# jedward225/MARL-HideAndSeek

Measured on AMD Instinct MI355X. Metric: world-steps/sec (agent-steps/sec derived) at 16K worlds, 1/2/4/8 GPU, higher is better.
Workload: dtype f32; 1 GPU; 16000 worlds/GPU x 2646 steps, 2 hiders + 2 seekers, sim_flags=0, rand_seed=0, random move actions in [-5,4] each step (scripts/benchmark.py args); worlds_per_gpu=16000, total_worlds=16000, agents_per_world=4

## Files before the change

### marl-hideandseek_amd/csrc/hs_k_observe.h

```cpp
#pragma once
#include "hs_state.h"
#include "hs_rays.h"

namespace hs {

constexpr int kObsWaves = 7;

constexpr int kRaysPerAgent = 46;
constexpr int obs_vis_base(int a) { return (a * 30 + 63) / 64 * 64; }
constexpr int obs_threads(int a) { return (obs_vis_base(a) + a * 16 + 63) / 64 * 64; }
constexpr int obs_max_agents(int nt) { int a = 1; while (a < kMaxAgents && obs_threads(a + 1) <= nt) ++a; return a; }
struct RayId { int agent, k; };
HSD RayId ray_id(int r, int visBase) {
    if (r < visBase) { const int i = r / 30; return {i, r - i * 30}; }
    const int rr = r - visBase;
    return {rr >> 4, 30 + (rr & 15)};
}

struct ObsStaged {
    WorldGeom g;
    float lin[kNumDSlots][3];
    float ang[kNumDSlots][3];
    int grab[kMaxAgents];
};

template <int NT>
struct ObsShared : ObsStaged {
    static constexpr int kMaxRays = NT, kAgents = obs_max_agents(NT);
    float rayD[kMaxRays][3];
    unsigned long long rayKey[kMaxRays];
    static constexpr int kWaves = NT / 64, kWavePairs = 64 * (kMaxBoxes + kMaxAgents - 1), kWaveRampPairs = 64 * kMaxRamps;
    unsigned short pairs[kWaves][kWavePairs];
    unsigned short rampPairs[kWaves][kWaveRampPairs];
    int nPairs[kWaves], nRampPairs[kWaves];
    unsigned present;
    alignas(16) float rel[kAgents][kNumDSlots][8];
    float fwd[kAgents][3], right[kAgents][3];
};

HSD void store_posvel(float *o, V3 p, V3 e, V3 l, V3 a) {
    o[0] = p.x; o[1] = p.y; o[2] = p.z; o[3] = e.x; o[4] = e.y; o[5] = e.z;
    o[6] = l.x; o[7] = l.y; o[8] = l.z; o[9] = a.x; o[10] = a.y; o[11] = a.z;
}

struct StageSeg { int rows, inner, stride, dst; };
enum { kStMeta, kStPos, kStRot, kStLin, kStAng, kStWall, kStPlane, kStGrab, kStSegs };
#define HS_ST_WORD(field) (int)(offsetof(ObsStaged, field) / 4)
#define HS_ST_GWORD(field) (int)((offsetof(ObsStaged, g) + offsetof(WorldGeom, field)) / 4)
constexpr StageSeg kStageSegs[kStSegs] = {
    {kNumDSlots, kNumDSlots, 1, HS_ST_GWORD(meta)},
    {3 * kNumDSlots, kNumDSlots, 3, HS_ST_GWORD(pos)},
    {4 * kNumDSlots, kNumDSlots, 4, HS_ST_GWORD(rot)},
    {3 * kNumDSlots, kNumDSlots, 3, HS_ST_WORD(lin)},
    {3 * kNumDSlots, kNumDSlots, 3, HS_ST_WORD(ang)},
    {4 * kMaxWalls, kMaxWalls, 4, HS_ST_GWORD(wall)},
    {4 * kMaxPlanes, kMaxPlanes, 4, HS_ST_GWORD(plane)},
    {kMaxAgents, kMaxAgents, 1, HS_ST_WORD(grab)},
};
constexpr int stage_seg_start(int k) { int f = 0; for (int j = 0; j < k; ++j) f += kStageSegs[j].rows; return f; }
constexpr int stage_seg_of(int f) { int k = 0; while (k + 1 < kStSegs && stage_seg_start(k + 1) <= f) ++k; return k; }
constexpr int kStageWords = stage_seg_start(kStSegs);
constexpr int kStagedWords = (int)(sizeof(ObsStaged) / 4);
struct StageTable { unsigned short dst[kStageWords]; };
constexpr StageTable make_stage_table() {
    StageTable t = {};
    int f = 0;
    for (int k = 0; k < kStSegs; ++k)
        for (int r = 0; r < kStageSegs[k].rows; ++r)
            t.dst[f++] = (unsigned short)((kStageSegs[k].dst + (r % kStageSegs[k].inner) * kStageSegs[k].stride + r / kStageSegs[k].inner) * 4);
    return t;
}
constexpr bool stage_table_covers() {
    const StageTable t = make_stage_table();
    int hits[kStagedWords] = {};
    for (int f = 0; f < kStageWords; ++f) {
        if (t.dst[f] % 4 != 0 || t.dst[f] / 4 >= kStagedWords) return false;
        ++hits[t.dst[f] / 4];
    }
    for (int w = 0; w < kStagedWords; ++w)
        if (hits[w] != (w == HS_ST_GWORD(numWalls) || w == HS_ST_GWORD(numPlanes) ? 0 : 1)) return false;
    return true;
}
static_assert(stage_table_covers(), "the staging table must write every staged word of ObsStaged exactly once");
static_assert(kStageWords == kNumDSlots + 3 * (3 * kNumDSlots) + 4 * kNumDSlots + 4 * kMaxWalls + 4 * kMaxPlanes + kMaxAgents,
              "the staging table moves the words of the per-column loops it replaced");
static_assert(kStagedWords == kStageWords + 2 && sizeof(ObsStaged) % 4 == 0, "ObsStaged holds the staged words and the two counts");
static_assert(kStageSegs[kStMeta].rows == decltype(SimState::bmeta)::kRows && kStageSegs[kStPos].rows == decltype(SimState::bpos)::kRows &&
              kStageSegs[kStRot].rows == decltype(SimState::brot)::kRows && kStageSegs[kStLin].rows == decltype(SimState::blin)::kRows &&
              kStageSegs[kStAng].rows == decltype(SimState::bang)::kRows && kStageSegs[kStWall].rows == decltype(SimState::walls)::kRows &&
              kStageSegs[kStPlane].rows == decltype(SimState::planes)::kRows && kStageSegs[kStGrab].rows == decltype(SimState::grabOther)::kRows,
              "every staged source row lies inside its column");
#undef HS_ST_WORD
#undef HS_ST_GWORD
__device__ const StageTable kStageTable = make_stage_table();

template <int NT>
HSD unsigned stage_world(const SimState &S, int ps, ObsShared<NT> &sh, int tid) {
    typedef unsigned __attribute__((may_alias)) word_t;
    const char *const arena = reinterpret_cast<const char *>(S.bpos.p);
    const void *const cols[kStSegs] = {S.bmeta.p, S.bpos.p, S.brot.p, S.blin.p, S.bang.p, S.walls.p, S.planes.p, S.grabOther.p};
    unsigned K[kStSegs];
#pragma unroll
    for (int k = 0; k < kStSegs; ++k)
        K[k] = (unsigned)(reinterpret_cast<const char *>(cols[k]) - arena) +
               (((unsigned)(ps >> 3) * kStageSegs[k].rows - stage_seg_start(k)) * kTile + (ps & 7)) * 4u;
    constexpr int kTrips = (kStageWords + NT - 1) / NT;
    unsigned v[kTrips], d[kTrips];
#pragma unroll
    for (int t = 0; t < kTrips; ++t) {
        const int f = tid + t * NT;
        const int lo = t * NT, hi = (t + 1) * NT < kStageWords ? (t + 1) * NT - 1 : kStageWords - 1;
        unsigned k = K[stage_seg_of(lo)];
#pragma unroll
        for (int s = 1; s < kStSegs; ++s)
            if (stage_seg_start(s) > lo && stage_seg_start(s) <= hi) k = f >= stage_seg_start(s) ? K[s] : k;
        v[t] = 0; d[t] = 0;
        if ((t + 1) * NT <= kStageWords || f < kStageWords) {
            v[t] = *reinterpret_cast<const word_t *>(arena + (size_t)(k + (unsigned)f * (kTile * 4u)));
            d[t] = kStageTable.dst[f];
        }
    }
    static_assert(kStageSegs[kStMeta].rows <= 64 && stage_seg_start(kStMeta) == 0, "the metas are staged by wave 0 in its first trip");
    const unsigned present = (unsigned)__ballot(tid < kNumDSlots && v[0] != 0);
    char *const dst = reinterpret_cast<char *>(static_cast<ObsStaged *>(&sh));
#pragma unroll
    for (int t = 0; t < kTrips; ++t)
        if ((t + 1) * NT <= kStageWords || tid + t * NT < kStageWords) *reinterpret_cast<word_t *>(dst + d[t]) = v[t];
    if (tid < NT / 64) { sh.nPairs[tid] = 0; sh.nRampPairs[tid] = 0; }
    return present;
}

HSD unsigned long long ray_key(float t, int id) { return ((unsigned long long)__float_as_uint(t) << 32) | (unsigned)id; }
constexpr unsigned kKeyMiss = 0xffffffffu;

template <int NT>
__global__ void __launch_bounds__(NT) __attribute__((amdgpu_waves_per_eu(kObsWaves, kObsWaves))) k_observe(SimState S) {
    __shared__ ObsShared<NT> sh;
    const int tid = threadIdx.x;
#ifdef HS_PHASE_TIMING
    long long otk = wall_clock64();
    long long *const oacc = S.phaseTicks + phase_ticks_obs_base(S.N) + (blockIdx.x & 1023) * 16;
#define HS_OTICK(i) { const long long now_ = wall_clock64(); if ((tid & 63) == 0) atomicAdd((unsigned long long *)&oacc[i], (unsigned long long)(now_ - otk)); otk = now_; }
#else
#define HS_OTICK(i)
#endif
    const int blk = blockIdx.x;
    int oct = ((blk >> 6) << 3) + (blk & 7);
    const int noct = (S.N + kTile - 1) / kTile;
    if (oct >= noct) return;
    if (step_serve(S) != kGroupAll) {
        if (oct >= *group_count(S, step_ring(S), step_serve(S))) return;
        oct = oct_list(S, step_ring(S), step_serve(S), noct)[oct];
    }
    const int p = oct * kTile + ((blk >> 3) & 7);
    const int4 hdr = S.slotHdr[p];
    const int A = S.A;
    const int visBase = obs_vis_base(A);
    const RayId myRay = ray_id(tid, visBase);
    float lidarS = 0.f, lidarC = 0.f;
    if (tid < visBase) { lidarS = S.lidarSinCos[myRay.k]; lidarC = S.lidarSinCos[30 + myRay.k]; }
    const unsigned present = stage_world<NT>(S, p, sh, tid);
    const int w = hdr.x;
    if (w < 0) return;
    if (tid == 0) { sh.g.numWalls = hdr.y & 255; sh.g.numPlanes = (hdr.y >> 8) & 255; sh.present = present; }
    const int counts = hdr.z;
    const int teams = hdr.w;
    const int step = hdr.y >> 16;
    __syncthreads();
    const WorldGeom &g = sh.g;
    const int nAgents = cnt_agents(counts), nBoxes = cnt_boxes(counts), nRamps = cnt_ramps(counts);
    HS_OTICK(0)
    static_assert(kNumDSlots - 1 == 16 && ObsShared<NT>::kAgents * 16 <= NT - 8, "item = agent * 16 + other body; the last 8 lanes have no item");
    for (int item = tid; item < nAgents * 16; item += NT) {
        const int i = item >> 4, ob = item & 15;
        const int b = ob + (ob >= kAgentSlot0 + i ? 1 : 0);
        const int m = g.meta[b];
        if (m == 0) continue;
        const V3 mo = g.g_pos(kAgentSlot0 + i) - g.g_pos(b);
        const V3 ol = qrot(qinv(g.g_rot(b)), mo);
        float *e = sh.rel[i][b];
        e[0] = mo.x; e[1] = mo.y; e[2] = mo.z;
        e[3] = dot(mo, mo) - obj_bound_r2(meta_obj(m));
        e[4] = ol.x; e[5] = ol.y; e[6] = ol.z;
    }
    for (int i = tid - (NT - 8); i >= 0 && i < nAgents; i += NT) {
        const Q rot = g.g_rot(kAgentSlot0 + i);
        const V3 f = qrot(rot, {0.f, 1.f, 0.f}), rt = qrot(rot, {1.f, 0.f, 0.f});
        sh.fwd[i][0] = f.x; sh.fwd[i][1] = f.y; sh.fwd[i][2] = f.z;
        sh.right[i][0] = rt.x; sh.right[i][1] = rt.y; sh.right[i][2] = rt.z;
    }
    __syncthreads();
    HS_OTICK(1)

    for (int r = tid; r < NT; r += NT) {
        const int i = myRay.agent, k = myRay.k;
        sh.rayKey[r] = ray_key(-1.f, kKeyMiss);
        if (i >= nAgents) continue;
        const int slot = kAgentSlot0 + i;
        const V3 o = g.g_pos(slot);
        const V3 fwd = {sh.fwd[i][0], sh.fwd[i][1], sh.fwd[i][2]};
        V3 d; float tmax;
        if (k < 30) {
            const V3 right = {sh.right[i][0], sh.right[i][1], sh.right[i][2]};
            const float s = lidarS, c = lidarC;
            d = normalize(right * c + fwd * s);
            tmax = 200.f;
        } else {
            const int e = k - 30;
            int tslot; bool present;
            if (e < kMaxBoxes) { tslot = kBoxSlot0 + e; present = e < nBoxes; }
            else if (e < kMaxBoxes + kMaxRamps) { tslot = kRampSlot0 + (e - kMaxBoxes); present = (e - kMaxBoxes) < nRamps; }
            else { const int jj = e - kMaxBoxes - kMaxRamps; const int j = jj < i ? jj : jj + 1; tslot = kAgentSlot0 + j; present = j < nAgents; }
            if (!present) continue;
            d = g.g_pos(tslot) - o;
            if (dot(normalize(d), fwd) < kCosFovHalf) continue;
            tmax = 1.f;
        }
        sh.rayD[r][0] = d.x; sh.rayD[r][1] = d.y; sh.rayD[r][2] = d.z;
        HS_OTICK(2)
        int hit = -1; float best = tmax;
        const V3 inv = {1.f / d.x, 1.f / d.y, 1.f / d.z};
// ... 64 lines not shown
        for (int v = 0; v < NW; ++v) { np2 += sh.nPairs[v]; nr2 += sh.nRampPairs[v]; }
        for (int p = tid; p < np2; p += NT) {
            int q = p, v = 0;
#pragma unroll
            for (int u = 0; u < NW - 1; ++u) { const int n = sh.nPairs[u]; if (v == u && q >= n) { q -= n; v = u + 1; } }
            const int pr = sh.pairs[v][q];
            const int r = pr >> 5, b = pr & 31;
            const int i = ray_id(r, visBase).agent;
            const float *e = sh.rel[i][b];
            const V3 ol = {e[4], e[5], e[6]};
            const V3 dl = qrot(qinv(g.g_rot(b)), {sh.rayD[r][0], sh.rayD[r][1], sh.rayD[r][2]});
            const V3 he = obj_half_extents(meta_obj(g.meta[b]));
            const float tmax = r < visBase ? 200.f : 1.f;
            const float t = __ballot(dl.x == 0.f || dl.y == 0.f || dl.z == 0.f) == 0 ? ray_box_local_nz(ol, dl, he) : ray_box_local(ol, dl, he);
            if (t >= 0.f && t <= tmax) atomicMin(&sh.rayKey[r], ray_key(t, b));
        }
        for (int p = NT - 1 - tid; p < nr2; p += NT) {
            int q = p, v = 0;
#pragma unroll
            for (int u = 0; u < NW - 1; ++u) { const int n = sh.nRampPairs[u]; if (v == u && q >= n) { q -= n; v = u + 1; } }
            const int pr = sh.rampPairs[v][q];
            const int r = pr >> 5, b = pr & 31;
            const int i = ray_id(r, visBase).agent;
            const float *e = sh.rel[i][b];
            const V3 dl = qrot(qinv(g.g_rot(b)), {sh.rayD[r][0], sh.rayD[r][1], sh.rayD[r][2]});
            const float tmax = r < visBase ? 200.f : 1.f;
            const float t = ray_wedge_local({e[4], e[5], e[6]}, dl);
            if (t >= 0.f && t <= tmax) atomicMin(&sh.rayKey[r], ray_key(t, b));
        }
    }
    __syncthreads();
    HS_OTICK(6)
    for (int r = tid; r < NT; r += NT) {
        const RayId rid = ray_id(r, visBase);
        const int i = rid.agent, k = rid.k;
        if (i >= nAgents) continue;
        const int row = w * A + i;
        const unsigned long long key = sh.rayKey[r];
        const unsigned id = (unsigned)(key & 0xffffffffull);
        const float t = __uint_as_float((unsigned)(key >> 32));
        if (k < 30) {
            S.xLidar[row * 30 + k] = id == kKeyMiss ? 0.f : t;
        } else {
            const int e = k - 30;
            if (e < kMaxBoxes) {
                S.xVisBoxes[row * kMaxBoxes + e] = (id == (unsigned)(kBoxSlot0 + e)) ? 1.f : 0.f;
            } else if (e < kMaxBoxes + kMaxRamps) {
                const int rr = e - kMaxBoxes;
                S.xVisRamps[row * kMaxRamps + rr] = (id == (unsigned)(kRampSlot0 + rr)) ? 1.f : 0.f;
            } else {
                const int jj = e - kMaxBoxes - kMaxRamps;
                const int j = jj < i ? jj : jj + 1;
                const float vis = (id == (unsigned)(kAgentSlot0 + j)) ? 1.f : 0.f;
                if (vis != 0.f && team_agent_type(teams, i) == AGENT_SEEKER && team_agent_type(teams, j) == AGENT_HIDER)
                    S.hiderTeamReward[w] = -1.f;
                S.xVisAgents[row * (kMaxAgents - 1) + jj] = vis;
            }
        }
    }
    HS_OTICK(7)
    const int nRel = A * 16, nObs = nRel + A;
    for (int item = tid; item < nObs + 1; item += NT) {
        if (item < nObs) {
            const int i = item < nRel ? item >> 4 : item - nRel, e = item < nRel ? 1 + (item & 15) : 0;
            if (i >= nAgents) continue;
            const int row = w * A + i;
            const int slot = kAgentSlot0 + i;
            const V3 mpos = g.g_pos(slot);
            const Q mrot = g.g_rot(slot);
            const V3 mlin = {sh.lin[slot][0], sh.lin[slot][1], sh.lin[slot][2]};
            const V3 mang = {sh.ang[slot][0], sh.ang[slot][1], sh.ang[slot][2]};
            const Q toF = qinv(mrot);
            if (e == 0) {
                if (step <= kNumPrepSteps) S.xPrep[row] = kNumPrepSteps - step;
                float *so = S.xSelfObs + row * 13;
                store_posvel(so, mpos, quat_to_euler(mrot), qrot(toF, mlin), qrot(toF, mang));
                so[12] = sh.grab[i] >= 0 ? 1.f : 0.f;
                continue;
            }
            int tslot; float *o; int width; bool present;
            if (e <= kMaxBoxes) {
                const int b = e - 1; tslot = kBoxSlot0 + b; width = 17; present = b < nBoxes;
                o = S.xBoxObs + (row * kMaxBoxes + b) * 17;
            } else if (e <= kMaxBoxes + kMaxRamps) {
                const int r = e - 1 - kMaxBoxes; tslot = kRampSlot0 + r; width = 14; present = r < nRamps;
                o = S.xRampObs + (row * kMaxRamps + r) * 14;
            } else {
                const int jj = e - 1 - kMaxBoxes - kMaxRamps;
                const int j = jj < i ? jj : jj + 1;
                tslot = kAgentSlot0 + j; width = 14; present = j < nAgents;
                o = S.xAgentObs + (row * (kMaxAgents - 1) + jj) * 14;
            }
            if (!present) { for (int k = 0; k < width; ++k) o[k] = 0.f; continue; }
            const V3 x = g.g_pos(tslot);
            const Q q = g.g_rot(tslot);
            const V3 lin = {sh.lin[tslot][0], sh.lin[tslot][1], sh.lin[tslot][2]};
            const V3 ang = {sh.ang[tslot][0], sh.ang[tslot][1], sh.ang[tslot][2]};
            V3 p = qrot(toF, x - mpos);
            Q qr = qnormalize(qmul(toF, q));
            store_posvel(o, p, quat_to_euler(qr), qrot(toF, lin - mlin), qrot(toF, ang - mang));
            const int m = g.meta[tslot];
            if (tslot < kAgentSlot0) {
                float *lk = o + (width - 2);
                if (tslot < kRampSlot0) {
                    const bool big = meta_obj(m) == OBJ_BOX;
                    o[12] = big ? 8.f : 2.f; o[13] = big ? 1.5f : 2.f; o[14] = 2.f;
                }
                if (meta_resp(m) != RESP_STATIC) { lk[0] = 0.f; lk[1] = 0.f; }
                else if (meta_owner(m) == OWNER_HIDER) { lk[0] = 1.f; lk[1] = 0.f; }
                else { lk[0] = 0.f; lk[1] = 1.f; }
            } else {
                const int j = tslot - kAgentSlot0;
                o[12] = team_agent_type(teams, j) == AGENT_HIDER ? 1.f : 0.f;
                o[13] = sh.grab[j] >= 0 ? 1.f : 0.f;
            }
        } else {
            float *gp = S.xGlobalPos + w * 34;
            for (int b = 0; b < kMaxBoxes; ++b) {
                bool on = b < nBoxes;
                gp[b * 2] = on ? g.pos[kBoxSlot0 + b][0] : 0.f; gp[b * 2 + 1] = on ? g.pos[kBoxSlot0 + b][1] : 0.f;
            }
            for (int r = 0; r < kMaxRamps; ++r) {
                bool on = r < nRamps;
                gp[18 + r * 2] = on ? g.pos[kRampSlot0 + r][0] : 0.f; gp[18 + r * 2 + 1] = on ? g.pos[kRampSlot0 + r][1] : 0.f;
            }
            float *ga = gp + 22;
// ... 18 lines not shown
```

### marl-hideandseek_amd/csrc/hs_k_physics.h

```cpp
#pragma once
#include "hs_state.h"
#include "hs_rays.h"
#include "hs_collide.h"
#include "hs_solver.h"
#include "hs_k_reset.h"

namespace hs {

constexpr int kPhysThreads = 64;
constexpr int kWorldLanes = kPhysThreads / kTile;
constexpr int kLdsWalls = 32;
static_assert(kMaxSCand <= 32 && kMaxDDCand <= 16, "accepted-manifold masks are one word per world");
constexpr int kAllDD = kNumDSlots * (kNumDSlots - 1) / 2;
constexpr int kAllSC = kNumDSlots * (kMaxWalls + kMaxPlanes - 1);
constexpr int kSpInfoWords = kNumDSlots + 1;

struct alignas(16) OctRes {
    static constexpr int kClip = kClipLanes;
    static constexpr int kClipWords = clip_words(kClip);
    static constexpr int kSatPairs = kClip < hs::kSatPairs ? kClip : hs::kSatPairs;
    static constexpr int kMaxItems = kTile * (kMaxDDCand + kMaxSCand);
    static constexpr int kSlots = kClip < 31 ? kClip : 31;
    static constexpr int kVelOffsetWords = 2 * 8 * 3 * 32;
    float pos[3][kNumDSlots][kTile];
    float rot[4][kNumDSlots][kTile];
    float ppos[3][kNumDSlots][kTile];
    float prot[4][kNumDSlots][kTile];
    int meta[kNumDSlots][kTile];
    union {
        struct {
            float lo[3][kNumDSlots][kTile], hi[3][kNumDSlots][kTile];
            float wall[4][kLdsWalls][kTile];
        } det;
        struct {
            float clip[kClipWords];
            unsigned short items[kMaxItems + 32];
            int pend[4][kClip];
        } sat;
        struct {
            float pad[kVelOffsetWords];
            float lin[3][kNumDSlots][kTile];
            float ang[3][kNumDSlots][kTile];
        } vel;
    } u;
    unsigned short ddPair[kMaxDDCand][kTile];
    unsigned short scPair[kMaxSCand][kTile];
    unsigned short scInfo[kNumDSlots][kTile];
    unsigned int scAcc[kTile];
    unsigned int ddAcc[kTile];
    unsigned int ddOrd[2][kTile];
    float plane0[4][kTile];
    unsigned char bodies[kNumDSlots * kTile];
    union {
        unsigned char wallBodies[kNumDSlots * kTile];
        unsigned char actGL[kMaxAgents][kTile];
    };
    unsigned int wallSeen[kTile];
    unsigned char numWalls[kTile], numPlanes[kTile], ndd[kTile], nsc[kTile], seen[kTile], hasGrab[kTile];
    unsigned char spill[kTile];
    int wid[kTile];
};
static_assert(sizeof(OctRes) <= 20 * 1024, "8 waves of 8 worlds share the CU's 160 KiB of LDS");
static_assert(offsetof(OctRes, u.sat.items) >= offsetof(OctRes, u.det.wall), "items must not overlap the AABBs");
static_assert(sizeof(ManDD) / 4 * OctRes::kSlots <= OctRes::kVelOffsetWords, "manifold slots lie below the velocities");
static_assert(2 * 3 * kNumDSlots * 8 <= OctRes::kVelOffsetWords, "the hull AABBs lie below the velocities");

constexpr int kLocGlobal = 31;
HSD int pair_a(int p) { return p & 31; }
HSD int pair_b(int p) { return (p >> 5) & 63; }
HSD int pair_loc(int p) { return (p >> 11) & 31; }
HSD int pair_pack(int a, int b) { return a | (b << 5) | (kLocGlobal << 11); }
static_assert(kNumDSlots <= 32 && kMaxWalls + kMaxPlanes <= 64, "pair encoding");
static_assert(sizeof(ManDD) % 16 == 0 && sizeof(ManS) % 16 == 0, "manifold records move 16 bytes at a time");
constexpr int kManWords = sizeof(ManDD) / 4;
template <typename M> HSD void man_lds_load(const float *clip, int slot, M &m) {
    m = *reinterpret_cast<const M *>(clip + slot * kManWords);
}
template <typename M> HSD void man_lds_set_lam(float *clip, int slot, int j, float v) {
    static_assert(offsetof(M, lam) == sizeof(M) - 16, "lam is the record's tail");
    clip[slot * kManWords + (sizeof(M) / 4 - 4 + j)] = v;
}

template <int C> HSD V3 rld3(const float (&a)[C][kNumDSlots][kTile], int slot, int g) { return {a[0][slot][g], a[1][slot][g], a[2][slot][g]}; }
HSD Q rld4(const float (&a)[4][kNumDSlots][kTile], int slot, int g) { return {a[0][slot][g], a[1][slot][g], a[2][slot][g], a[3][slot][g]}; }
HSD void rst3(float (&a)[3][kNumDSlots][kTile], int slot, int g, V3 v) { a[0][slot][g] = v.x; a[1][slot][g] = v.y; a[2][slot][g] = v.z; }
HSD void rst4(float (&a)[4][kNumDSlots][kTile], int slot, int g, Q q) { a[0][slot][g] = q.w; a[1][slot][g] = q.x; a[2][slot][g] = q.y; a[3][slot][g] = q.z; }

HSD void rbody_load(const OctRes &R, int g, int slot, BodyS &b) {
    b.pos = rld3(R.pos, slot, g); b.rot = rld4(R.rot, slot, g);
    b.ppos = rld3(R.ppos, slot, g); b.prot = rld4(R.prot, slot, g);
    b.lin = rld3(R.u.vel.lin, slot, g); b.ang = rld3(R.u.vel.ang, slot, g);
    const int m = R.meta[slot][g];
    const bool dyn = m != 0 && meta_resp(m) == RESP_DYNAMIC;
    b.invM = dyn ? obj_inv_mass(meta_obj(m)) : 0.f;
    b.invI = dyn ? obj_inv_inertia(meta_obj(m)) : V3{0.f, 0.f, 0.f};
    body_refresh_inertia(b);
}
HSD void rbody_store_pose(OctRes &R, int g, int slot, const BodyS &b) { rst3(R.pos, slot, g, b.pos); rst4(R.rot, slot, g, b.rot); }
HSD void rbody_store_vel(OctRes &R, int g, int slot, const BodyS &b) { rst3(R.u.vel.lin, slot, g, b.lin); rst3(R.u.vel.ang, slot, g, b.ang); }
HSD void derive_velocity(BodyS &b) {
    const float h = kSubstepH;
    b.lin = (b.pos - b.ppos) * (1.f / h);
    Q dq = qmul(b.rot, qinv(b.prot));
    V3 wv = V3{dq.x, dq.y, dq.z} * (2.f / h);
    b.ang = dq.w >= 0.f ? wv : -wv;
}

HSD void wave_sync() { asm volatile("s_waitcnt lgkmcnt(0)" ::: "memory"); }
HSD void mem_sync() { asm volatile("s_waitcnt vmcnt(0) lgkmcnt(0)" ::: "memory"); }

template <int D> HSD int dpp_row_shr(int x) { return __builtin_amdgcn_update_dpp(0, x, 0x110 + D, 0xF, 0xF, true); }
HSD int scan8_incl(int x, int l) {
    int y;
    y = dpp_row_shr<1>(x); if (l >= 1) x += y;
// ... 945 lines not shown
    }
}

HSD void phase_pre(const SimState &S, OctRes &R) {
    const int A_ = S.A, L = hs_lane();
    const bool instant = (S.flags & FLAG_ZERO_AGENT_VELOCITY) == FLAG_ZERO_AGENT_VELOCITY;
    bool need_action = false;
    if (L < kMaxAgents * kTile) {
        const int agent = L / kTile, g = L % kTile;
        const int w = R.wid[g], p = S.wbeg + g;
        int fl = 0;
        if (agent < A_ && w >= 0) {
            const int teams = S.teams[w], step = S.curEpisodeStep[w];
            const bool active = team_agent_active(teams, agent) != 0;
            const int type = team_agent_type(teams, agent);
            if (active && !(type == AGENT_SEEKER && step < kNumPrepSteps - 1)) {
                int32_t *act_row = S.xAction + (w * A_ + agent) * 5;
                const int ax = act_row[0], ay = act_row[1], ar = act_row[2], ag = act_row[3], al = act_row[4];
                float fx, fy, tz;
                if (instant) { fx = 400.f * (float)(ax - 2); fy = 400.f * (float)(ay - 2); tz = 120.f * (float)(ar - 2); }
                else { fx = 12.f * (float)(ax - 5); fy = 12.f * (float)(ay - 5); tz = 3.f * (float)(ar - 5); }
                V3 f = qrot(rld4(R.rot, kAgentSlot0 + agent, g), {fx, fy, 0.f});
                S.aforce(0 * kMaxAgents + agent, p) = f.x; S.aforce(1 * kMaxAgents + agent, p) = f.y;
                S.aforce(2 * kMaxAgents + agent, p) = f.z; S.aforce(3 * kMaxAgents + agent, p) = tz;
                fl = (ag == 1 ? 1 : 0) | (al == 1 ? 2 : 0);
                act_row[0] = 2; act_row[1] = 2; act_row[2] = 2; act_row[3] = 0; act_row[4] = 0;
            }
        }
        R.actGL[agent][g] = (unsigned char)fl;
        need_action = fl != 0;
    }
    const bool any = __ballot(need_action) != 0ull;
    wave_sync();
    if (any && L < kTile && R.wid[L] >= 0) {
        bool want = false;
        for (int a = 0; a < A_; ++a) want |= R.actGL[a][L] != 0;
        if (want) action_system(S, R, L, A_, S.teams[R.wid[L]]);
    }
    if (L < kTile) {
        bool grab = false;
        if (R.wid[L] >= 0) for (int a = 0; a < kMaxAgents; ++a) grab |= S.grabOther(a, S.wbeg + L) >= 0;
        R.hasGrab[L] = grab ? 1 : 0;
    }
    wave_sync();
}

HSD void phase_post(const SimState &S, OctRes &R) {
    constexpr int G = kWorldLanes;
    const int L = hs_lane(), g = L / G, l = L % G;
    const int w = R.wid[g], p = S.wbeg + g;
    const int A_ = S.A;
    const bool wok = w >= 0;
    const bool instant = (S.flags & FLAG_ZERO_AGENT_VELOCITY) == FLAG_ZERO_AGENT_VELOCITY;
    int teams = 0, step = 0, counts = 0;
    if (wok) {
        teams = S.teams[w]; step = S.curEpisodeStep[w]; counts = S.counts[w];
        if (l == 0) R.seen[g] = 0;
        if (instant && l < kMaxAgents && R.meta[kAgentSlot0 + l][g] != 0) {
            const int slot = kAgentSlot0 + l;
            R.u.vel.lin[0][slot][g] = 0.f; R.u.vel.lin[1][slot][g] = 0.f;
            R.u.vel.lin[2][slot][g] = fminf(R.u.vel.lin[2][slot][g], 0.f);
            rst3(R.u.vel.ang, slot, g, V3{0.f, 0.f, 0.f});
        }
    }
    wave_sync();
    for (int pr = l; wok && step >= kNumPrepSteps - 1 && pr < 9; pr += G) {
        const int si = pr / 3, hi_ = pr % 3;
        if (si < cnt_seekers(counts) && hi_ < cnt_hiders(counts)) {
            const ResGeom geom = {R, S, g, p};
            const int ss = kAgentSlot0 + team_seeker(teams, si), hs_ = kAgentSlot0 + team_hider(teams, hi_);
            const V3 spos = geom.g_pos(ss);
            const V3 fwd = qrot(geom.g_rot(ss), {0.f, 1.f, 0.f});
            V3 to = geom.g_pos(hs_) - spos;
            float c = dot(normalize(to), fwd);
            if (!(c < kCosFovHalf)) {
                float t;
                if (trace_ray(geom, spos, to, 1.f, &t) == hs_) R.seen[g] = 1;
            }
        }
    }
    wave_sync();
    if (!wok) return;
    float hider_reward = S.hiderTeamReward[w];
    if (R.seen[g]) hider_reward = -1.f;
    if (l < A_ && team_agent_active(teams, l)) {
        const int agent = l, slot = kAgentSlot0 + agent, row = w * A_ + agent;
        if (step == 0) S.xDone[row] = 0;
        if (step < kNumPrepSteps - 1) {
            S.xReward[row] = 0.f;
        } else {
            if (step == kEpisodeLen - 1) S.xDone[row] = 1;
            float r = hider_reward;
            if (team_agent_type(teams, agent) == AGENT_SEEKER) r *= -1.f;
            if (fabsf(R.pos[0][slot][g]) >= 18.f || fabsf(R.pos[1][slot][g]) >= 18.f) r -= 10.f;
            S.xReward[row] = r;
        }
    }
    if (l == 0) {
        float *res = S.xEpisodeResult + w * 2;
        int s0 = S.runningScores(0, p), s1 = S.runningScores(1, p);
        if (step == 0) { res[0] = 0.f; res[1] = 0.f; s0 = 0; s1 = 0; }
        if (step >= kNumPrepSteps) {
            const bool hidden = hider_reward == 1.f;
            const bool sf = cnt_seekers_first(counts) != 0;
            const int win = hidden ? (sf ? 1 : 0) : (sf ? 0 : 1);
            if (win == 0) s0 += 1; else s1 += 1;
        }
        if (step == kEpisodeLen - 1) {
            if (s0 > s1) { res[0] = 1.f; res[1] = 0.f; }
            else if (s0 < s1) { res[0] = 0.f; res[1] = 1.f; }
            else { res[0] = 0.5f; res[1] = 0.5f; }
        }
        S.runningScores(0, p) = s0; S.runningScores(1, p) = s1;
        S.hiderTeamReward[w] = hider_reward;
    }
}

template <int ROUNDS, int LASTR, bool POS>
HSD void static_passes(const SimState &S, OctRes &R, BodyReg (&br)[ROUNDS], int nbodies, int nLast, int nMerged) {
    const int L = hs_lane();
#pragma unroll
    for (int r = 0; r < LASTR; ++r) {
        const bool valid = r * 64 + L < nbodies; const int t_ = valid ? R.bodies[r * 64 + L] : 0;
        const int slot = t_ >> 3, g = t_ & 7; const int meta = valid ? R.meta[slot][g] : 0;
        if (valid) { if (POS) ground_pos(R, br[r], slot, g, meta); else ground_vel(R, br[r], slot, g, meta); }
    }
    wave_sync();
    {
        const bool valid = LASTR * 64 + L < nbodies; const int t_ = valid ? R.bodies[LASTR * 64 + L] : 0;
        const int slot = t_ >> 3, g = t_ & 7; const int meta = valid ? R.meta[slot][g] : 0;
        last_round<POS>(S, R, br[LASTR], valid, slot, g, meta, nLast, nMerged);
    }
    wave_sync();
}

#ifdef HS_PHASE_TIMING
#define HS_TICK_PARAMS , long long &tk, long long (&acc)[10]
// ... 96 lines not shown
    HS_TICK(0)
    int nbodies;
    {
        int base = 0;
#pragma unroll
        for (int pass = 0; pass < 2; ++pass) {
#pragma unroll
            for (int c = 0; c < ROUNDS; ++c) {
                const int t = c * 64 + L;
                const int ord = t / kTile, g = t % kTile;
                const int slot = ord < S.A ? kAgentSlot0 + ord : ord - S.A;
                const bool hist = ord < NS && ((R.wallSeen[g] >> slot) & 1u) != 0u;
                const bool on = ord < NS && R.meta[slot][g] != 0 && hist == (pass == 0);
                const unsigned long long m = __ballot(on);
                if (on) R.bodies[base + __popcll(m & ((1ull << L) - 1ull))] = (unsigned char)(slot << 3 | g);
                base += __popcll(m);
            }
        }
        nbodies = base;
    }
    wave_sync();
    if (L < kTile) R.wallSeen[L] = 0u;
    wave_sync();
    BodyReg br[ROUNDS];
    const float *const aforce = S.aforce.octet(p0 >> 3);
#pragma unroll
    for (int r = 0; r < ROUNDS; ++r) {
        BodyReg &b = br[r];
        b.np = 0; b.vidx = 0;
#pragma unroll
        for (int j = 0; j < 4; ++j) b.lam[j] = 0.f;
        HS_BODY(r)
        if (valid) integrate_body(R, b, slot, g, meta, aforce);
    }
    wave_sync();
    HS_TICK(1)
#pragma unroll 1
    for (int sub = 0; sub < kNumSubsteps; ++sub) {
        const ItemCounts ic = phase_detect<ROUNDS>(S, R, NS);
        HS_TICK(2)
        substep_rest<ROUNDS>(S, R, br, nbodies, NS, ic, sub + 1 < kNumSubsteps, aforce HS_TICK_ARGS);
    }
#undef HS_BODY
    phase_post(S, R);
    wave_sync();
    copy_out(S.bpos, p0, &R.pos[0][0][0]); copy_out(S.brot, p0, &R.rot[0][0][0]);
    copy_out_vel(S.blin, p0, &R.u.vel.lin[0][0][0], R); copy_out_vel(S.bang, p0, &R.u.vel.ang[0][0][0], R);
    copy_out(S.bmeta, p0, &R.meta[0][0]);
    mem_sync();
    HS_TICK(8)
    {
        const int myWorld = L < kTile ? R.wid[L] : -1;
        const int mySeen = L < kTile ? (int)R.wallSeen[L] : 0;
        wave_sync();
        if (myWorld >= 0) {
            S.wallHist[myWorld] = mySeen;
            reset_world(S, myWorld, gen[L]);
        }
    }
    if (L == 0) {
        const int dt = (int)(wall_clock64() - tStart);
        S.octTicks[o] = dt;
        atomicAdd(&S.tickSum[sidx], (unsigned long long)dt);
        const int group = dt + prevTicks > lateAbove ? kGroupLate : kGroupEarly;
        oct_list(S, nextIdx, group, noct)[atomicAdd(group_count(S, nextIdx, group), 1)] = o;
    }
#ifdef HS_PHASE_TIMING
    if (L == 0) for (int i = 0; i < 10; ++i) S.phaseTicks[(size_t)o * 10 + i] += acc[i];
#endif
#undef HS_TICK
}

template <int ROUNDS>
__global__ void __launch_bounds__(kPhysThreads, 2) k_physics(SimState S) {
    __shared__ union PhysLds { OctRes R; GenScratch gen[kTile]; } lds;
    static_assert(sizeof(PhysLds) <= 20 * 1024, "8 waves of 8 worlds share the CU's 160 KiB of LDS");
    physics_step<ROUNDS>(S, lds.R, lds.gen);
}

}
```

### marl-hideandseek_amd/csrc/hs_k_reset.h

```cpp
#pragma once
#include "../../include/hideseek.h"
#include "hs_state.h"

namespace hs {

struct Seg { float x1, y1, x2, y2; };

HSD Seg seg_make(float ax, float ay, float bx, float by) {
    if (ax > bx || ay > by) return {bx, by, ax, ay};
    return {ax, ay, bx, by};
}
HSD void seg_resort(Seg &s) {
    if (s.x1 > s.x2 || s.y1 > s.y2) { Seg t = s; s = {t.x2, t.y2, t.x1, t.y1}; }
}
HSD bool seg_horizontal(const Seg &s) { return fabsf(s.y1 - s.y2) < 0.000001f; }
HSD float seg_length(const Seg &s) { return seg_horizontal(s) ? (s.x2 - s.x1) : (s.y2 - s.y1); }

struct WallSet {
    Seg segs[kMaxWalls]; int n;
    uint8_t horiz[kMaxWalls]; int nh;
    uint8_t vert[kMaxWalls]; int nv;
};
HSD int wallset_add(WallSet &w, Seg s) {
    if (w.n >= kMaxWalls) return w.n - 1;
// ... 339 lines not shown
        teams |= (g.agentType[i] & 1) << (18 + i);
        if (i < g.numActiveAgents) teams |= 1 << (24 + i);
        S.grabOther(i, ps) = -1;
        for (int c = 0; c < 4; ++c) S.aforce(c * kMaxAgents + i, ps) = 0.f;
    }
    S.teams[w] = teams;
    S.counts[w] = cnt_pack(g.numHiders, g.numSeekers, g.numActiveAgents, g.numActiveBoxes, g.numActiveRamps, g.seekersFirst);
    const int A = S.A;
    for (int i = 0; i < A; ++i) {
        int row = w * A + i;
        if (i < g.numActiveAgents) {
            S.xSelfType[row] = g.agentType[i];
            S.xSelfMask[row] = 1.f;
            S.xSeed[row * 2 + 0] = (int32_t)ep; S.xSeed[row * 2 + 1] = (int32_t)world_id;
            int32_t *a = S.xAction + row * 5;
            a[0] = 2; a[1] = 2; a[2] = 2; a[3] = 0; a[4] = 0;
        } else {
            S.xSelfMask[row] = 0.f;
        }
    }
    if (!LOAD) return;
    S.runningScores(0, ps) = ck->running_scores[0]; S.runningScores(1, ps) = ck->running_scores[1];
    auto put_body = [&](int slot, const float *b) {
        for (int c = 0; c < 3; ++c) {
            S.bpos(c * kNumDSlots + slot, ps) = b[c];
            S.blin(c * kNumDSlots + slot, ps) = b[7 + c];
            S.bang(c * kNumDSlots + slot, ps) = b[10 + c];
        }
        for (int c = 0; c < 4; ++c) S.brot(c * kNumDSlots + slot, ps) = b[3 + c];
    };
    const int nb = ck->num_boxes < 0 ? 0 : (ck->num_boxes > g.numActiveBoxes ? g.numActiveBoxes : ck->num_boxes);
    const int nr = ck->num_ramps < 0 ? 0 : (ck->num_ramps > g.numActiveRamps ? g.numActiveRamps : ck->num_ramps);
    for (int i = 0; i < nb + nr; ++i) {
        const hs_ckpt_object &o = i < nb ? ck->boxes[i] : ck->ramps[i - nb];
        const int slot = i < nb ? i : kRampSlot0 + (i - nb);
        put_body(slot, o.pos);
        S.bmeta(slot, ps) = meta_pack(g.obj[slot], o.is_locked ? RESP_STATIC : RESP_DYNAMIC, (int)(o.team & 3u));
    }
    for (int i = 0; i < g.numHiders + g.numSeekers; ++i) {
        const hs_ckpt_agent &a = ck->agents[i];
        const int ai = i < g.numHiders ? g.hiders[i] : g.seekers[i - g.numHiders];
        put_body(kAgentSlot0 + ai, a.pos);
        if (a.grab_idx >= 0 && a.grab_idx < nb + nr) {
            S.grabOther(ai, ps) = a.grab_idx < nb ? a.grab_idx : kRampSlot0 + (a.grab_idx - nb);
            float gd[kGrabWords] = {a.grab_r2[0], a.grab_r2[1], a.grab_r2[2],
                                    a.attach_rot2[0], a.attach_rot2[1], a.attach_rot2[2], a.attach_rot2[3], a.separation,
                                    a.grab_r1[0], a.grab_r1[1], a.grab_r1[2],
                                    a.attach_rot1[0], a.attach_rot1[1], a.attach_rot1[2], a.attach_rot1[3]};
            for (int c = 0; c < kGrabWords; ++c) S.grabData(c * kMaxAgents + ai, ps) = gd[c];
        }
    }
}

HSD void write_slot_hdr(const SimState &S, int w, int ps) {
    const int step = S.curEpisodeStep[w];
    S.slotHdr[ps] = make_int4(w, S.numWalls[w] | (S.numPlanes[w] << 8) | ((step < 0x7fff ? step : 0x7fff) << 16), S.counts[w], S.teams[w]);
}

HSD void reset_world(const SimState &S, int w, GenScratch &scratch) {
    int level = S.xReset[w];
    const int step = S.curEpisodeStep[w];
    if ((S.flags & FLAG_IGNORE_EPISODE_LENGTH) != FLAG_IGNORE_EPISODE_LENGTH && step == kEpisodeLen - 1) level = 1;
    if (level == 0) {
        S.curEpisodeStep[w] = step + 1;
        S.hiderTeamReward[w] = 1.f;
        write_slot_hdr(S, w, S.slotOfWorld[w]);
        return;
    }
    regenerate_world<false>(S, w, level, nullptr, scratch);
    write_slot_hdr(S, w, S.slotOfWorld[w]);
}

__global__ void __launch_bounds__(64) k_reset(SimState S) {
    const int w = blockIdx.x * blockDim.x + threadIdx.x;
    if (w >= S.N) return;
    GenScratch scratch;
    reset_world(S, w, scratch);
}

__global__ void __launch_bounds__(64) k_lidar_table(SimState S) {
    const int k = threadIdx.x;
    if (k >= 30) return;
    const float theta = 2.f * kPi * ((float)k / 30.f) + kPi / 2.f;
    hs_sincosf(theta, &S.lidarSinCos[k], &S.lidarSinCos[30 + k]);
}

__global__ void __launch_bounds__(64) k_load_ckpt(SimState S) {
    const int w = blockIdx.x * blockDim.x + threadIdx.x;
    if (w >= S.N) return;
    if (S.xCkptCtrl[w] == 0) return;
    S.xCkptCtrl[w] = 1;
    GenScratch scratch;
    regenerate_world<true>(S, w, 1, (const hs_checkpoint *)S.xCkpt + w, scratch);
    write_slot_hdr(S, w, S.slotOfWorld[w]);
}

__global__ void __launch_bounds__(64) k_save_ckpt(SimState S) {
    const int w = blockIdx.x * blockDim.x + threadIdx.x;
    const int N = S.N;
    if (w >= N) return;
    if (S.xCkptCtrl[w] == 0) return;
    S.xCkptCtrl[w] = 0;
    const int ps = S.slotOfWorld[w];
    hs_checkpoint *ck = (hs_checkpoint *)S.xCkpt + w;
    uint32_t *raw = (uint32_t *)ck;
    for (int i = 0; i < (int)(sizeof(hs_checkpoint) / 4); ++i) raw[i] = 0u;
    ck->episode_key[0] = S.epKeyA[w]; ck->episode_key[1] = S.epKeyB[w];
    ck->running_scores[0] = S.runningScores(0, ps); ck->running_scores[1] = S.runningScores(1, ps);
    ck->episode_step = S.curEpisodeStep[w];
    const int cnt = S.counts[w], teams = S.teams[w];
    const int nh = cnt_hiders(cnt), ns = cnt_seekers(cnt), nb = cnt_boxes(cnt), nr = cnt_ramps(cnt);
    auto get_body = [&](int slot, float *b) {
        for (int c = 0; c < 3; ++c) {
            b[c] = S.bpos(c * kNumDSlots + slot, ps);
            b[7 + c] = S.blin(c * kNumDSlots + slot, ps);
            b[10 + c] = S.bang(c * kNumDSlots + slot, ps);
        }
        for (int c = 0; c < 4; ++c) b[3 + c] = S.brot(c * kNumDSlots + slot, ps);
    };
// ... 30 lines not shown
```

### marl-hideandseek_amd/csrc/hs_state.h

```cpp
#pragma once
#include "hs_dev.h"

namespace hs {

constexpr int kTile = 8;
template <typename T, int ROWS> struct Col {
    T *p;
    static constexpr int kRows = ROWS;
    HSD T &operator()(int row, int w) const { return p[((size_t)(w >> 3) * ROWS + row) * kTile + (w & 7)]; }
    HSD T *octet(int o) const { return p + (size_t)o * ROWS * kTile; }
};

struct SimState {
    int N;
    int A;
    uint32_t flags;
    RandKey initKey;
    int minHiders, maxHiders, minSeekers, maxSeekers;
    int worldOffset;
    int wbeg, wcnt;
    int *slotOfWorld;
    int *worldOfSlot;
    int *loadAcc;
    int *wallHist;
    int4 *slotHdr;
    int *octTicks;
    unsigned long long *tickSum;
    int stepIdx;
    float *lidarSinCos;

    Col<float, 3 * kNumDSlots> bpos;
    Col<float, 4 * kNumDSlots> brot;
    Col<float, 3 * kNumDSlots> blin;
    Col<float, 3 * kNumDSlots> bang;
    Col<int, kNumDSlots> bmeta;
    Col<float, 4 * kMaxAgents> aforce;
    Col<float, 4 * kMaxWalls> walls;
    Col<float, 4 * kMaxPlanes> planes;
    int *numWalls;
    int *numPlanes;
    uint32_t *curWorldEpisode;
    uint32_t *rngKeyA, *rngKeyB, *rngCount;
    uint32_t *epKeyA, *epKeyB;
    int *curEpisodeStep;
    float *hiderTeamReward;
    int *counts;
    int *teams;
    Col<int, 2> runningScores;
    Col<int, kMaxAgents> grabOther;
    Col<float, kGrabWords * kMaxAgents> grabData;

    int32_t *xReset, *xPrep, *xAction, *xSelfType, *xSeed, *xDone, *xPolicy;
    float *xSelfObs, *xSelfMask, *xAgentObs, *xBoxObs, *xRampObs, *xVisAgents, *xVisBoxes, *xVisRamps;
    float *xLidar, *xReward, *xGlobalPos, *xEpisodeResult;
    int32_t *xCkptCtrl;
    uint8_t *xCkpt;
    void *wsDD, *wsSC;
    unsigned short *spPair;
    int *spInfo;
    int *status;
    long long *phaseTicks;
};

constexpr int kGroupAll = -1, kGroupEarly = 0, kGroupLate = 1;
constexpr int kSchedBase = 32, kSchedFactor = 0, kCountStride = 32, kSchedCounts = 32, kSchedLists = kSchedCounts + 6 * kCountStride;
__host__ __device__ inline int step_idx_arg(int ring, int serve) { return ring | (serve + 1) << 2; }
__host__ __device__ inline int step_ring(const SimState &S) { return S.stepIdx & 3; }
__host__ __device__ inline int step_serve(const SimState &S) { return (S.stepIdx >> 2) - 1; }
__host__ __device__ inline int *sched_words(const SimState &S) { return reinterpret_cast<int *>(S.tickSum) + kSchedBase; }
__host__ __device__ inline size_t sched_alloc_sums(int noct) { return ((size_t)kSchedBase + kSchedLists + (size_t)6 * noct + 1) / 2; }
__host__ __device__ inline int *group_count(const SimState &S, int idx, int group) { return sched_words(S) + kSchedCounts + (idx * 2 + group) * kCountStride; }
__host__ __device__ inline int *oct_list(const SimState &S, int idx, int group, int noct) { return sched_words(S) + kSchedLists + (size_t)(idx * 2 + group) * noct; }

__host__ __device__ inline size_t phase_ticks_obs_base(int N) { return (size_t)10 * ((N + kTile - 1) / kTile); }

HSD int cnt_hiders(int c) { return c & 15; }
HSD int cnt_seekers(int c) { return (c >> 4) & 15; }
HSD int cnt_agents(int c) { return (c >> 8) & 15; }
HSD int cnt_boxes(int c) { return (c >> 12) & 15; }
HSD int cnt_ramps(int c) { return (c >> 16) & 15; }
HSD int cnt_seekers_first(int c) { return (c >> 20) & 1; }
HSD int cnt_pack(int nh, int ns, int na, int nb, int nr, int sf) {
    return nh | (ns << 4) | (na << 8) | (nb << 12) | (nr << 16) | (sf << 20);
}
HSD int team_hider(int t, int i) { return (t >> (3 * i)) & 7; }
HSD int team_seeker(int t, int i) { return (t >> (9 + 3 * i)) & 7; }
HSD int team_agent_type(int t, int i) { return (t >> (18 + i)) & 1; }
HSD int team_agent_active(int t, int i) { return (t >> (24 + i)) & 1; }

}
```

Measured before the change: 33.98 million world-steps/s.

## Defer seeker-hider visibility test from physics to observation ray results

Physics no longer runs its own seeker-to-hider line-of-sight checks when observations will be computed anyway. It marks the world as deferred in a high bit of the slot header. The observe kernel then reuses its agent-visibility ray hits to settle rewards and running scores when a seeker sees a hider, and clears the mark. This removes duplicated visibility raycasting in physics but couples reward correctness to the observation pass. It also adds an atomic and extra global writes in observe.

```diff
diff --git a/marl-hideandseek_amd/csrc/hs_k_observe.h b/marl-hideandseek_amd/csrc/hs_k_observe.h
--- a/marl-hideandseek_amd/csrc/hs_k_observe.h
+++ b/marl-hideandseek_amd/csrc/hs_k_observe.h
@@ -34,6 +34,8 @@
     unsigned short rampPairs[kWaves][kWaveRampPairs];
     int nPairs[kWaves], nRampPairs[kWaves];
     unsigned present;
+    int sawHider;
+    int slot;
     alignas(16) float rel[kAgents][kNumDSlots][8];
     float fwd[kAgents][3], right[kAgents][3];
 };
@@ -134,6 +136,21 @@
 constexpr unsigned kKeyMiss = 0xffffffffu;
 
 template <int NT>
+HSD void settle_deferred_reward(const SimState &S, ObsShared<NT> &sh, int w, int step, int counts, int teams) {
+    const int A = S.A, nAgents = cnt_agents(counts);
+    for (int a = 0; a < nAgents; ++a) {
+        float r = -1.f;
+        if (team_agent_type(teams, a) == AGENT_SEEKER) r *= -1.f;
+        if (fabsf(sh.g.pos[kAgentSlot0 + a][0]) >= 18.f || fabsf(sh.g.pos[kAgentSlot0 + a][1]) >= 18.f) r -= 10.f;
+        S.xReward[w * A + a] = r;
+    }
+    if (atomicExch(&sh.sawHider, 1) == 0 && step >= kNumPrepSteps + 1) {
+        const int ps = sh.slot, hiddenWin = cnt_seekers_first(counts) != 0 ? 1 : 0;
+        S.runningScores(hiddenWin, ps) -= 1; S.runningScores(1 - hiddenWin, ps) += 1;
+    }
+}
+
+template <int NT>
 __global__ void __launch_bounds__(NT) __attribute__((amdgpu_waves_per_eu(kObsWaves, kObsWaves))) k_observe(SimState S) {
     __shared__ ObsShared<NT> sh;
     const int tid = threadIdx.x;
@@ -162,11 +179,13 @@
     const unsigned present = stage_world<NT>(S, p, sh, tid);
     const int w = hdr.x;
     if (w < 0) return;
-    if (tid == 0) { sh.g.numWalls = hdr.y & 255; sh.g.numPlanes = (hdr.y >> 8) & 255; sh.present = present; }
+    if (tid == 0) { sh.g.numWalls = hdr.y & 255; sh.g.numPlanes = (hdr.y >> 8) & 255; sh.present = present; sh.sawHider = 0; sh.slot = p; }
     const int counts = hdr.z;
     const int teams = hdr.w;
-    const int step = hdr.y >> 16;
+    static_assert(kHdrDeferred == 1u << 31, "the mark is the sign of the header's second word");
+    const int stepMark = hdr.y >> 16;
     __syncthreads();
+    if (tid == 0 && stepMark < 0) S.slotHdr[p].y = hdr.y & 0x7fffffff;
     const WorldGeom &g = sh.g;
     const int nAgents = cnt_agents(counts), nBoxes = cnt_boxes(counts), nRamps = cnt_ramps(counts);
     HS_OTICK(0)
@@ -337,8 +356,10 @@
                 const int jj = e - kMaxBoxes - kMaxRamps;
                 const int j = jj < i ? jj : jj + 1;
                 const float vis = (id == (unsigned)(kAgentSlot0 + j)) ? 1.f : 0.f;
-                if (vis != 0.f && team_agent_type(teams, i) == AGENT_SEEKER && team_agent_type(teams, j) == AGENT_HIDER)
+                if (vis != 0.f && team_agent_type(teams, i) == AGENT_SEEKER && team_agent_type(teams, j) == AGENT_HIDER) {
                     S.hiderTeamReward[w] = -1.f;
+                    if (stepMark < 0) settle_deferred_reward(S, sh, w, stepMark & 0x7fff, counts, teams);
+                }
                 S.xVisAgents[row * (kMaxAgents - 1) + jj] = vis;
             }
         }
@@ -357,6 +378,7 @@
             const V3 mang = {sh.ang[slot][0], sh.ang[slot][1], sh.ang[slot][2]};
             const Q toF = qinv(mrot);
             if (e == 0) {
+                const int step = stepMark & 0x7fff;
                 if (step <= kNumPrepSteps) S.xPrep[row] = kNumPrepSteps - step;
                 float *so = S.xSelfObs + row * 13;
                 store_posvel(so, mpos, quat_to_euler(mrot), qrot(toF, mlin), qrot(toF, mang));
diff --git a/marl-hideandseek_amd/csrc/hs_k_physics.h b/marl-hideandseek_amd/csrc/hs_k_physics.h
--- a/marl-hideandseek_amd/csrc/hs_k_physics.h
+++ b/marl-hideandseek_amd/csrc/hs_k_physics.h
@@ -60,6 +60,7 @@
     unsigned char spill[kTile];
     int wid[kTile];
 };
+constexpr int kSeenDeferred = 2;
 static_assert(sizeof(OctRes) <= 20 * 1024, "8 waves of 8 worlds share the CU's 160 KiB of LDS");
 static_assert(offsetof(OctRes, u.sat.items) >= offsetof(OctRes, u.det.wall), "items must not overlap the AABBs");
 static_assert(sizeof(ManDD) / 4 * OctRes::kSlots <= OctRes::kVelOffsetWords, "manifold slots lie below the velocities");
@@ -1111,9 +1112,11 @@
     const int A_ = S.A;
     const bool wok = w >= 0;
     const bool instant = (S.flags & FLAG_ZERO_AGENT_VELOCITY) == FLAG_ZERO_AGENT_VELOCITY;
-    int teams = 0, step = 0, counts = 0;
+    int teams = 0, step = 0, counts = 0, resetReq = 0;
+    float hider_reward = 0.f;
     if (wok) {
         teams = S.teams[w]; step = S.curEpisodeStep[w]; counts = S.counts[w];
+        hider_reward = S.hiderTeamReward[w]; resetReq = S.xReset[w];
         if (l == 0) R.seen[g] = 0;
         if (instant && l < kMaxAgents && R.meta[kAgentSlot0 + l][g] != 0) {
             const int slot = kAgentSlot0 + l;
@@ -1122,8 +1125,12 @@
             rst3(R.u.vel.ang, slot, g, V3{0.f, 0.f, 0.f});
         }
     }
-    wave_sync();
-    for (int pr = l; wok && step >= kNumPrepSteps - 1 && pr < 9; pr += G) {
+    const bool undecided = wok && step >= kNumPrepSteps - 1 && hider_reward != -1.f;
+    const bool defer = undecided && (S.flags & FLAG_EXT_SKIP_OBSERVATIONS) != FLAG_EXT_SKIP_OBSERVATIONS && resetReq == 0 &&
+                       !((S.flags & FLAG_IGNORE_EPISODE_LENGTH) != FLAG_IGNORE_EPISODE_LENGTH && step == kEpisodeLen - 1);
+    if (defer && l == 0) R.seen[g] = kSeenDeferred;
+    wave_sync();
+    for (int pr = l; undecided && !defer && pr < 9; pr += G) {
         const int si = pr / 3, hi_ = pr % 3;
         if (si < cnt_seekers(counts) && hi_ < cnt_hiders(counts)) {
             const ResGeom geom = {R, S, g, p};
@@ -1140,8 +1147,7 @@
     }
     wave_sync();
     if (!wok) return;
-    float hider_reward = S.hiderTeamReward[w];
-    if (R.seen[g]) hider_reward = -1.f;
+    if (R.seen[g] == 1) hider_reward = -1.f;
     if (l < A_ && team_agent_active(teams, l)) {
         const int agent = l, slot = kAgentSlot0 + agent, row = w * A_ + agent;
         if (step == 0) S.xDone[row] = 0;
@@ -1344,10 +1350,11 @@
     {
         const int myWorld = L < kTile ? R.wid[L] : -1;
         const int mySeen = L < kTile ? (int)R.wallSeen[L] : 0;
+        const bool myDeferred = L < kTile && R.seen[L] == kSeenDeferred;
         wave_sync();
         if (myWorld >= 0) {
             S.wallHist[myWorld] = mySeen;
-            reset_world(S, myWorld, gen[L]);
+            reset_world(S, myWorld, gen[L], myDeferred);
         }
     }
     if (L == 0) {
diff --git a/marl-hideandseek_amd/csrc/hs_k_reset.h b/marl-hideandseek_amd/csrc/hs_k_reset.h
--- a/marl-hideandseek_amd/csrc/hs_k_reset.h
+++ b/marl-hideandseek_amd/csrc/hs_k_reset.h
@@ -415,19 +415,21 @@
     }
 }
 
-HSD void write_slot_hdr(const SimState &S, int w, int ps) {
+HSD void write_slot_hdr(const SimState &S, int w, int ps, bool deferred = false) {
     const int step = S.curEpisodeStep[w];
-    S.slotHdr[ps] = make_int4(w, S.numWalls[w] | (S.numPlanes[w] << 8) | ((step < 0x7fff ? step : 0x7fff) << 16), S.counts[w], S.teams[w]);
-}
-
-HSD void reset_world(const SimState &S, int w, GenScratch &scratch) {
+    const unsigned y = (unsigned)S.numWalls[w] | ((unsigned)S.numPlanes[w] << 8) | ((unsigned)(step < 0x7fff ? step : 0x7fff) << 16) |
+                       (deferred ? kHdrDeferred : 0u);
+    S.slotHdr[ps] = make_int4(w, (int)y, S.counts[w], S.teams[w]);
+}
+
+HSD void reset_world(const SimState &S, int w, GenScratch &scratch, bool deferred = false) {
     int level = S.xReset[w];
     const int step = S.curEpisodeStep[w];
     if ((S.flags & FLAG_IGNORE_EPISODE_LENGTH) != FLAG_IGNORE_EPISODE_LENGTH && step == kEpisodeLen - 1) level = 1;
     if (level == 0) {
         S.curEpisodeStep[w] = step + 1;
         S.hiderTeamReward[w] = 1.f;
-        write_slot_hdr(S, w, S.slotOfWorld[w]);
+        write_slot_hdr(S, w, S.slotOfWorld[w], deferred);
         return;
     }
     regenerate_world<false>(S, w, level, nullptr, scratch);
diff --git a/marl-hideandseek_amd/csrc/hs_state.h b/marl-hideandseek_amd/csrc/hs_state.h
--- a/marl-hideandseek_amd/csrc/hs_state.h
+++ b/marl-hideandseek_amd/csrc/hs_state.h
@@ -62,6 +62,8 @@
     long long *phaseTicks;
 };
 
+constexpr unsigned kHdrDeferred = 1u << 31;
+
 constexpr int kGroupAll = -1, kGroupEarly = 0, kGroupLate = 1;
 constexpr int kSchedBase = 32, kSchedFactor = 0, kCountStride = 32, kSchedCounts = 32, kSchedLists = kSchedCounts + 6 * kCountStride;
 __host__ __device__ inline int step_idx_arg(int ring, int serve) { return ring | (serve + 1) << 2; }
```

Measured after the change: 34.66 million world-steps/s, median of 6. 1.02x the previous value.
